# bioinfo-ut/GenomeTester4

Measured on AMD Instinct MI355X. Metric: k-mers merged/sec, 2-list k=25 intersection (glistcompare -i), lists resident in HBM, higher is better.
Workload: dtype u64 keys + u32 counts

## Files before the change

genometester4_amd/csrc/gt4hip_api.hip:

```cpp
#include "gt4hip_host.h"

#include <stdarg.h>
#include <stdio.h>
#include <stdlib.h>
#include <string.h>
#include <new>

using namespace gt4;

static thread_local char g_create_err[512] = "";

static void pool_flush (gt4hip_context *ctx);

int gt4hip_fail (gt4hip_context *ctx, int code, const char *fmt, ...)
{
  va_list ap;
  va_start (ap, fmt);
  vsnprintf (ctx ? ctx->err : g_create_err, 512, fmt, ap);
  va_end (ap);
  return code;
}

extern "C" const char *gt4hip_strerror (int code)
{
// ... 111 lines not shown
  if (!ctx) return GT4HIP_EINVAL;
  HIPCHK (ctx, hipSetDevice (ctx->device));
  HIPCHK (ctx, hipStreamSynchronize (ctx->stream));
  pool_flush (ctx);
  return GT4HIP_OK;
}

extern "C" int gt4hip_device_memory (gt4hip_context *ctx, uint64_t *free_bytes, uint64_t *total_bytes)
{
  if (!ctx) return GT4HIP_EINVAL;
  HIPCHK (ctx, hipSetDevice (ctx->device));
  size_t f = 0, t = 0;
  HIPCHK (ctx, hipMemGetInfo (&f, &t));
  if (free_bytes) *free_bytes = (uint64_t) f + ctx->pool_bytes;
  if (total_bytes) *total_bytes = (uint64_t) t;
  return GT4HIP_OK;
}

extern "C" int gt4hip_set_option (gt4hip_context *ctx, const char *name, int64_t value)
{
  if (!ctx || !name) return GT4HIP_EINVAL;
  if (!strcmp (name, "two_pass")) ctx->two_pass = value != 0;
  else if (!strcmp (name, "pool")) {
    ctx->pool_enabled = value != 0 && ctx->pool;
    if (!ctx->pool_enabled) pool_flush (ctx);
  }
  else if (!strcmp (name, "pool_cap_mb")) {
    ctx->pool_cap = value > 0 ? (size_t) value << 20 : 0;
    if (ctx->pool_bytes > ctx->pool_cap) pool_flush (ctx);
  }
  else if (!strcmp (name, "grid")) ctx->grid_override = value;
  else if (!strcmp (name, "scan_group")) ctx->scan_group = (int) value;
  else if (!strcmp (name, "dynamic")) ctx->dynamic = (int) value;
  else if (!strcmp (name, "kway")) ctx->kway_enabled = (int) value;
  else if (!strcmp (name, "kway_max")) ctx->kway_max = value == 8 ? 8 : (value == 33 ? 33 : 32);
  else if (!strcmp (name, "kway_g")) ctx->kway_g = value;
  else if (!strcmp (name, "kway_vt")) ctx->kway_vt = value;
  else if (!strcmp (name, "spin_limit")) ctx->spin_limit = value > 0 ? (uint32_t) value : 0u;
  else if (!strcmp (name, "geom1")) ctx->force_geom = value != 0 ? 1 : 0;
  else if (!strcmp (name, "geom0")) ctx->force_geom = value != 0 ? -1 : 0;
  else return gt4hip_fail (ctx, GT4HIP_EINVAL, "unknown option %s", name);
  return GT4HIP_OK;
}

extern "C" int gt4hip_get_counter (gt4hip_context *ctx, const char *name, uint64_t *value)
{
  if (!ctx || !name || !value) return GT4HIP_EINVAL;
  if (!strcmp (name, "single_pass_fallbacks")) *value = ctx->single_pass_fallbacks;
  else if (!strcmp (name, "kway_calls")) *value = ctx->kway_calls;
  else if (!strcmp (name, "kway_overflows")) *value = ctx->kway_overflows;
  else if (!strcmp (name, "kway_declined")) *value = ctx->kway_declined;
  else if (!strcmp (name, "kway_splits")) *value = ctx->kway_splits;
  else if (!strcmp (name, "kway_shared_x100")) *value = ctx->kway_shared_x100;
  else if (!strcmp (name, "kway_width")) *value = ctx->kway_width;
  else if (!strcmp (name, "nway_kernel_us")) *value = (uint64_t) (ctx->nway_kernel_ms * 1000.0);
  else if (!strcmp (name, "nway_tiles")) *value = ctx->nway_tiles;
  else if (!strcmp (name, "nway_one_pass")) *value = (uint64_t) ctx->last_multi_one_pass;
  else if (!strcmp (name, "sort_us")) *value = (uint64_t) (ctx->sort_ms * 1000.0);
  else if (!strcmp (name, "fold_us")) *value = (uint64_t) (ctx->fold_ms * 1000.0);
  else if (!strcmp (name, "extract_us")) *value = (uint64_t) (ctx->extract_ms * 1000.0);
  else if (!strcmp (name, "maker_text_tile") || !strcmp (name, "maker_code_tile")) *value = GT4HIP_MAKER_TILE;
  else if (!strcmp (name, "table_us")) *value = (uint64_t) (ctx->table_ms * 1000.0);
  else if (!strcmp (name, "query_wide")) *value = ctx->query_wide;
  else if (!strcmp (name, "mm_wide_levels")) *value = ctx->mm_wide_levels;
  else if (!strcmp (name, "mm_unskipped_levels")) *value = ctx->mm_unskipped_levels;
  else return gt4hip_fail (ctx, GT4HIP_EINVAL, "unknown counter %s", name);
// ... 310 lines not shown
```

genometester4_amd/csrc/gt4hip_device.h:

```cpp
#ifndef GT4HIP_DEVICE_H
#define GT4HIP_DEVICE_H

#include "gt4hip_internal.h"

namespace gt4 {
namespace {

constexpr int WAVE = 64;

typedef unsigned long long u64;
typedef unsigned int u32;
typedef u32 u32x4 __attribute__ ((ext_vector_type (4)));


__device__ __forceinline__ u64 load_key (const u32 *__restrict__ rec, u64 i)
{
  const u32 *p = rec + 3 * i;
  return (u64) p[0] | ((u64) p[1] << 32);
}



__device__ __forceinline__ u64 shfl_up_u64 (u64 v, int d)
{
// ... 10 lines not shown
__device__ __forceinline__ u64 wave_inclusive_scan (u64 v, int lane)
{
#pragma unroll
  for (int d = 1; d < WAVE; d <<= 1) {
    const u64 o = shfl_up_u64 (v, d);
    if (lane >= d) v += o;
  }
  return v;
}

__device__ __forceinline__ u64 wave_sum (u64 v)
{
#pragma unroll
  for (int m = WAVE / 2; m > 0; m >>= 1) v += shfl_xor_u64 (v, m);
  return v;
}

__device__ __forceinline__ u32 dpp_inclusive_scan_u32 (u32 v)
{
  v += (u32) __builtin_amdgcn_update_dpp (0, (int) v, 0x111, 0xf, 0xf, false);
  v += (u32) __builtin_amdgcn_update_dpp (0, (int) v, 0x112, 0xf, 0xf, false);
  v += (u32) __builtin_amdgcn_update_dpp (0, (int) v, 0x114, 0xf, 0xf, false);
  v += (u32) __builtin_amdgcn_update_dpp (0, (int) v, 0x118, 0xf, 0xf, false);
  v += (u32) __builtin_amdgcn_update_dpp (0, (int) v, 0x142, 0xa, 0xf, false);
  v += (u32) __builtin_amdgcn_update_dpp (0, (int) v, 0x143, 0xc, 0xf, false);
  return v;
}

__device__ __forceinline__ u32 dpp_wave_sum_u32 (u32 v)
{
  return (u32) __builtin_amdgcn_readlane ((int) dpp_inclusive_scan_u32 (v), WAVE - 1);
}

template <int NCH>
__device__ __forceinline__ u32 chunk_scan (u64 *km, u32 *cp, int lane)
{
  static_assert (NCH <= 2 * WAVE, "two chunks per lane");
  const u32 v0 = lane < NCH ? (u32) __popcll (km[lane]) : 0u;
  const u32 v1 = (NCH > WAVE && lane + WAVE < NCH) ? (u32) __popcll (km[NCH > WAVE ? lane + WAVE : 0]) : 0u;
  const u32 incl = dpp_inclusive_scan_u32 (v0 | (v1 << 16));
  const u32 last = (u32) __builtin_amdgcn_readlane ((int) incl, WAVE - 1);
  const u32 t0 = last & 0xffffu, total = t0 + (last >> 16);
  if (lane < NCH) cp[lane] = (incl & 0xffffu) - v0;
  if (NCH > WAVE && lane + WAVE < NCH) cp[lane + WAVE] = t0 + (incl >> 16) - v1;
  if (lane == 0) {
    cp[NCH] = total;
    km[NCH] = 0;
  }
  return total;
}


constexpr u32 AGG_READY = 1u << 31;
constexpr u64 CARRY_READY = 1ull << 63;

__device__ __forceinline__ void publish_u32 (u32 *p, u32 v) { __hip_atomic_store (p, v, __ATOMIC_RELAXED, __HIP_MEMORY_SCOPE_AGENT); }
__device__ __forceinline__ void publish_u64 (u64 *p, u64 v) { __hip_atomic_store (p, v, __ATOMIC_RELAXED, __HIP_MEMORY_SCOPE_AGENT); }
__device__ __forceinline__ u32 peek_u32 (u32 *p) { return __hip_atomic_load (p, __ATOMIC_RELAXED, __HIP_MEMORY_SCOPE_AGENT); }
__device__ __forceinline__ u64 peek_u64 (u64 *p) { return __hip_atomic_load (p, __ATOMIC_RELAXED, __HIP_MEMORY_SCOPE_AGENT); }

#define GT4_STAMP_TID GT4_PROFILE_PHASES
#define PHASE_STAMP(i) PROF (do { __builtin_amdgcn_sched_barrier (0); u64 t_; asm volatile ("s_memtime %0\n\ts_waitcnt lgkmcnt(0)" : "=s"(t_) :: "memory"); __builtin_amdgcn_sched_barrier (0); if (tid == GT4_STAMP_TID) { ph[i] += t_ - t_last; } t_last = t_; } while (0))

constexpr u32 SPIN_LIMIT = 1u << 22;
#define GT4_SCAN_ROWS 16
constexpr int SCAN_ROWS = GT4_SCAN_ROWS;

__device__ void scanner_wave (u32 *agg, u64 *carry_out, u64 num_tiles, PairControl *ctl, int lane, u32 spin_limit)
{
  __builtin_amdgcn_s_setprio (3);
  u64 carry = 0;
  const u64 rows = (num_tiles + WAVE - 1) / WAVE;
  if (lane == 0) publish_u64 (&carry_out[0], CARRY_READY);
  u32 v[SCAN_ROWS], w[SCAN_ROWS];
  auto load_batch = [&] (u32 (&dst)[SCAN_ROWS], u64 r0) {
#pragma unroll
    for (int j = 0; j < SCAN_ROWS; j++) {
      const u64 idx = (r0 + j) * WAVE + lane;
// ... 247 lines not shown
```

genometester4_amd/csrc/gt4hip_host.h:

```cpp
#ifndef GT4HIP_HOST_H
#define GT4HIP_HOST_H

#include "../../include/gt4hip.h"
#include "gt4hip_internal.h"

#include <stddef.h>
#include <algorithm>
#include <utility>
#include <vector>

struct gt4hip_io;

struct gt4hip_context {
  int device;
  hipStream_t stream;
  hipEvent_t ev[4];
  int n_cus;
  int two_pass;
  int64_t grid_override;
  uint32_t spin_limit;
  int dynamic;
  int scan_group;
  int force_geom;
  uint64_t single_pass_fallbacks;
  std::vector<std::pair<void *, size_t>> *pool;
  int pool_enabled;
  size_t pool_bytes;
  size_t pool_cap;
  uint64_t *part;
  size_t part_bytes;
  unsigned long long *desc;
  size_t desc_bytes;
  unsigned long long *block_sums;
  size_t block_sums_bytes;
  gt4::PairControl *ctl;
  gt4::PairControl *ctl_host;
  unsigned long long *scratch;
  unsigned long long *scratch_host;
  uint64_t *kway_part;
  size_t kway_part_bytes;
  void *kway_cnt;
  size_t kway_cnt_bytes;
  uint64_t *kway_part2;
  size_t kway_part2_bytes;
  void *kway_need;
  size_t kway_need_bytes;
  uint64_t kway_splits;
  int kway_enabled;
  int kway_max;
  uint64_t kway_width;
  uint64_t kway_shared_x100;
  int64_t kway_g;
  int64_t kway_vt;
// ... 104 lines not shown
```

genometester4_amd/csrc/gt4hip_kernels.hip:

```cpp
#define GT4_RESOLVE_LOOKBACK 3
#include "gt4hip_device.h"

#include <type_traits>

namespace gt4 {

namespace {


enum : u32 { KIND_SKIP = 0, KIND_A = 1, KIND_B = 2, KIND_BOTH = 3 };

struct StreamCoef {
  u32 m_f1, m_f2, m_min, m_max, m_sub2;
  u32 konst;
  u32 minz;
  u32 check_in;
  u32 lo;
  u32 cutoff;
  u32 subtract;
};

template <int S>
__device__ __forceinline__ StreamCoef make_coef (const PairParams &p)
{
// ... 107 lines not shown

template <int NT, int IPT, int OPS>
struct RankShared {
  static constexpr int CAP = NT * IPT;
  static constexpr int NCH = CAP / WAVE;
  static constexpr int STAGE_DW = OPS == STAGE_INTRSEC ? ((3 * (CAP / 2 + 1) + 3) & ~3)
                                  : ((OPS == STAGE_UNION || OPS == STAGE_COMPLEMENT) ? 3 * CAP
                                     : (OPS == STAGE_ANY ? 3 * (2 * CAP + 16) : (OPS == STAGE_UNION_LATE ? 3 * (CAP + 16) : 4)));
  static constexpr int STAGE_SLOTS = (OPS == STAGE_INTRSEC && IPT <= 4 && NT > 512) ? 4 : ((OPS == STAGE_ANY || OPS == STAGE_UNION_LATE) ? 1 : 2);
  alignas (16) u32 raw[3 * CAP];
  u32 stage[STAGE_SLOTS][STAGE_DW];
  u64 kmask[4][NCH + 1];
  u32 cpre[4][NCH + 1];
  u64 excl[4];
  u32 tot[4];
  u32 tick[3];
  u64 rng[3][4];
  u32 tile_id[3];
  u64 trash[WAVE];
};

__device__ __forceinline__ void store_lane0 (u64 *dst, u64 *trash, u64 v, int lane)
{
  u64 *const w = lane == 0 ? dst : trash + lane;
  *w = v;
}

__device__ __forceinline__ u32 kept_before (const u64 *km, const u32 *cp, u32 z)
{
  const u32 c = z >> 6;
  return cp[c] + (u32) __popcll (km[c] & ((1ull << (z & 63u)) - 1ull));
}

template <int S, int NT, int IPT, int OPS, int FAST, class Shared>
__device__ __forceinline__ void scatter_stream (Shared &sh, u32 *dst32, const PairParams &p, u32 nbs, int lane, int wid,
                                                const u64 (&key)[IPT], const u32 (&fa)[IPT], const u32 (&fb)[IPT], const u32 (&meta)[IPT])
{
  constexpr int NW = NT / WAVE;
  const StreamCoef c = make_coef<S> (p);
  constexpr bool A_ONLY = S == 1 || S == 2;
  const u32 pna = A_ONLY ? 0u : kept_before (sh.kmask[S], sh.cpre[S], nbs);
#pragma unroll
  for (int k = 0; k < IPT; k++) {
    const u32 chunk = (u32) k * NW + (u32) wid;
    const u64 mv = sh.kmask[S][chunk];
    const u32 m_lo = __builtin_amdgcn_readfirstlane ((u32) mv), m_hi = __builtin_amdgcn_readfirstlane ((u32) (mv >> 32));
    if (__builtin_amdgcn_inverse_ballot_w64 (((u64) m_hi << 32) | m_lo)) {
      const u32 own = sh.cpre[S][chunk] + __builtin_amdgcn_mbcnt_hi (m_hi, __builtin_amdgcn_mbcnt_lo (m_lo, 0u));
      u32 slot = own;
      if (!A_ONLY) {
        const u32 r = meta[k] & 0xffffu;
        const u32 z = ((meta[k] >> 18) & 1u) ? nbs + r : r;
        slot += kept_before (sh.kmask[S], sh.cpre[S], z) - pna;
      }
      u32 f;
      if (OPS != 0) f = fa[k];
      else if (FAST) eval_default<S> ((meta[k] >> 16) & 3u, fa[k], fb[k], p.cutoff, f);
      else eval_stream<S> ((meta[k] >> 16) & 3u, fa[k], fb[k], c, f);
      dst32[3 * slot] = (u32) key[k];
      dst32[3 * slot + 1] = (u32) (key[k] >> 32);
      dst32[3 * slot + 2] = f;
    }
  }
}

template <int CAP, int G>
__device__ __forceinline__ void rank_group (const u32 *lds32, const u32 (&sbase)[G], const u32 (&sn)[G], const u64 (&ky)[G], u32 (&lo)[G], bool narrow, u32 base_lo)
{
  auto key_at = [&] (u32 byte_off) -> u64 {
    const u32 *const q = reinterpret_cast<const u32 *> (reinterpret_cast<const char *> (lds32) + byte_off);
    return (u64) q[0] | ((u64) q[1] << 32);
  };
  constexpr u32 HTOP = (CAP & (CAP - 1)) ? (1u << (31 - __builtin_clz ((unsigned) CAP))) / 2 : CAP / 4;
  u32 at[G];
  auto step = [&] (u32 h) {
    u64 pv[G];
// ... 82 lines not shown
  for (int u = 0; u < G; u++) lo[u] = at[u] - 4u * sbase[u];
}

struct TileRange {
  u64 a0, b0;
  u32 na, nb;
};


template <int NT, int IPT, int MODE, int OPS, int FAST = 0, int OPSET = 0>
__global__ __launch_bounds__ (NT, merge_waves_per_simd (NT, MODE, OPS, FAST)) void
k_pair_merge (const u32 *__restrict__ A, u64 nA, const u32 *__restrict__ B, u64 nB, u64 *part, u64 num_tiles,
              PairParams p, PairOutputs outs, u64 *desc, PairControl *ctl)
{
  constexpr int CAP = NT * IPT;
  constexpr int NW = NT / WAVE;
  constexpr int NCH = CAP / WAVE;
  constexpr int NLOAD4 = (3 * IPT + 3) / 4;
  constexpr bool LATE1 = OPS == 1 && IPT > 4;
  constexpr bool DEFER = OPS != 0 && !LATE1 && MODE != MODE_COUNT;
  constexpr int S0 = OPS == 2 ? 1 : (OPS == 4 ? 2 : 0);
  static_assert (OPS == 0 || OPS == 1 || OPS == 2 || OPS == 4, "specialised kernels exist for one of these outputs alone");
  constexpr bool GDEFER = (OPS == 0 || LATE1) && MODE != MODE_COUNT;
  constexpr int G = IPT % 3 == 0 ? 3 : 2;
  constexpr int F_TOP = GDEFER ? NLOAD4 + 1 : (OPS == 4 ? NLOAD4 : (OPS == 2 ? 2 : 1));
  constexpr int F_MID = (GDEFER || OPS == 4 || OPS == 2) ? 0 : 1;
  constexpr bool STAGGER = NT >= 1024;
  static_assert (NW >= 4, "one wavefront per output stream in phase 2");
  static_assert (NCH <= 2 * WAVE, "chunk scan is a single wavefront pass");
  typedef RankShared<NT, IPT, (MODE == MODE_COUNT ? STAGE_NONE : (OPS == 0 ? STAGE_ANY : (OPS == 4 ? STAGE_COMPLEMENT : (OPS == 2 ? STAGE_INTRSEC : (IPT > 4 ? STAGE_UNION_LATE : STAGE_UNION)))))> Shared;
  __shared__ Shared sh;
  u32 *const lds32 = sh.raw;

  constexpr bool OPAQUE_TID = OPS == 0 && !(FAST == 1 && (OPSET == 3 || OPSET == 5) && MODE != MODE_COUNT);
  int tid = threadIdx.x, lane = tid & (WAVE - 1);
  const int wid = __builtin_amdgcn_readfirstlane (tid / WAVE);
  static_assert (pair_variant_exists ({ NT, IPT, MODE, OPS, FAST, OPSET }), "not an instantiation the selection can return (a compile-time stream set belongs to the any-combination kernel)");
  const u32 ops = OPS ? (u32) OPS : (OPSET ? (u32) OPSET : p.ops);
  const bool need_b = (ops & 9u) != 0;

  const u64 n_rows = (num_tiles + WAVE - 1) / WAVE;
  const u32 spin_limit = p.spin_limit ? p.spin_limit : SPIN_LIMIT;
  u32 *const agg = reinterpret_cast<u32 *> (desc);
  u64 *const carry = desc + 2 * n_rows * WAVE;

  u32 role = 0;
  if (MODE == MODE_LOOKBACK) {
    if (tid == 0) sh.tick[0] = atomicAdd (&ctl->role, 1u);
    __syncthreads ();
    role = sh.tick[0];
    __syncthreads ();
    if (role == 0) {
      const u32 n_str = (u32) __builtin_popcount (ops);
      const u32 k = (u32) wid % n_str, sub = (u32) wid / n_str, n_sub = ((u32) NW - k + n_str - 1) / n_str;
      u32 s = 0;
      for (u32 seen = 0, b = 0; b < 4; b++)
        if ((ops >> b) & 1u) {
          if (seen == k) s = b;
          seen++;
        }
      u64 *const rowsum = carry + 4 * (n_rows + 1);
      if (sub < 8u && (p.scan_group || sub == 0))
        scanner_part (agg + (u64) s * n_rows * WAVE, rowsum + (u64) s * n_rows, carry + (u64) s * (n_rows + 1), num_tiles, ctl, lane, spin_limit, sub,
                      p.scan_group ? (n_sub > 8u ? 8u : n_sub) : 1u);
      return;
    }
  }
// ... 148 lines not shown
    if (DEFER && w_have) {
      constexpr int WK = (Shared::STAGE_DW / 4 + NT - 1) / NT;
      write_out_fixed<NT, WK> (outs.rec[S0], uniform64 (sh.excl[S0]), w_tot, sh.stage[it % LAG], tid);
    }
    u32 xagg = 0;
    u64 xcarry = 0;
    if (GDEFER && MODE == MODE_LOOKBACK && it >= 1 && wid >= 4 && wid < 8 && ((ops >> (wid - 4)) & 1u)) {
      const int s = wid - 4;
      const u32 pt = past[LAG - 1];
      const u64 prow = pt / WAVE;
      if ((u32) lane < pt % WAVE) xagg = peek_u32 (&agg[(u64) s * n_rows * WAVE + prow * WAVE + lane]);
      xcarry = peek_u64 (&carry[(u64) s * (n_rows + 1) + prow]);
    }
    if (nxt < ntl) {
      if (STAGGER) {
#pragma unroll
        for (int j = 0; j < F_TOP; j++) fetch_part (tn, j);
      } else fetch (tn);
    }

    bool narrow = false;
    u32 base_lo = 0;
    if (OPS == 2 && MODE != MODE_COUNT && na && nb) {
      const u32 la = 3 * (na - 1), lb = OB + 3 * (nb - 1);
      const u64 a_min = (u64) lds32[0] | ((u64) lds32[1] << 32), a_max = (u64) lds32[la] | ((u64) lds32[la + 1] << 32);
      const u64 b_min = (u64) lds32[OB] | ((u64) lds32[OB + 1] << 32), b_max = (u64) lds32[lb] | ((u64) lds32[lb + 1] << 32);
      const u64 t_min = a_min < b_min ? a_min : b_min, t_max = a_max > b_max ? a_max : b_max;
      narrow = __builtin_amdgcn_ballot_w64 (((t_max - t_min) >> 32) == 0) != 0;
      base_lo = (u32) t_min;
    }
    PHASE_STAMP (2);
    u64 key[IPT];
    u32 fa[IPT], fb[IPT], meta[IPT];
    {
      const StreamCoef c0 = make_coef<0> (p), c1 = make_coef<1> (p), c2 = make_coef<2> (p), c3 = make_coef<3> (p);
      static_assert (IPT % G == 0, "chunks are searched in groups");
#pragma unroll
      for (int kk = 0; kk < IPT; kk += G) {
        if (STAGGER && kk == G && nxt < ntl) {
#pragma unroll
          for (int j = F_TOP; j < F_TOP + F_MID; j++) fetch_part (tn, j);
        }
        bool live[G], valid[G], any_live = false;
        u32 is_a[G], own[G], lim[G], lo[G];
        u32 sbase[G], sn[G];
        u32 plim[G];
        u64 ky[G];
#pragma unroll
        for (int u = 0; u < G; u++) {
          const u32 cbeg = ((u32) (kk + u) * NW + (u32) wid) * WAVE;
          is_a[u] = cbeg < nbs ? 1u : 0u;
          plim[u] = is_a[u] ? na : (need_b ? npos : 0u);
          live[u] = cbeg < plim[u];
          any_live |= live[u];
        }
        if (!any_live) {
#pragma unroll
          for (int u = 0; u < G; u++) {
            const int k = kk + u;
            key[k] = 0;
            fa[k] = fb[k] = 0;
            meta[k] = KIND_SKIP << 16;
            {
              const u32 chunk = (u32) k * NW + (u32) wid;
#pragma unroll
              for (int s = 0; s < 4; s++)
                if ((ops >> s) & 1u) store_lane0 (&sh.kmask[s][chunk], sh.trash, 0ull, lane);
            }
          }
          continue;
        }
#pragma unroll
        for (int u = 0; u < G; u++) {
          const u32 e = (u32) (kk + u) * NT + (u32) tid;
          u32 at;
          if (OPS == 2) {
            valid[u] = live[u] && (is_a[u] ? e < na : e < npos);
            at = valid[u] ? (is_a[u] ? 3 * e : OB + 3 * (e - nbs)) : 0u;
          } else {
            valid[u] = e < plim[u];
            const u32 off = is_a[u] ? 0u : OB - 3 * nbs;
            at = valid[u] ? 3 * e + off : 0u;
          }
          ky[u] = (u64) lds32[at] | ((u64) lds32[at + 1] << 32);
          own[u] = lds32[at + 2];
          sbase[u] = is_a[u] ? OB : 0u;
          sn[u] = is_a[u] ? nb : na;
          lim[u] = valid[u] ? 12 * sn[u] : 0u;
          lo[u] = 0;
        }
        rank_group<CAP, G> (lds32, sbase, sn, ky, lo, narrow, base_lo);
#pragma unroll
        for (int u = 0; u < G; u++) {
          const int k = kk + u;
          const u32 chunk = (u32) k * NW + (u32) wid;
          const u32 r = (lo[u] * 43691u) >> 19;
          const bool in = lo[u] < lim[u];
          const u32 oat = sbase[u] + (in ? lo[u] >> 2 : 0u);
          const u64 okey = (u64) lds32[oat] | ((u64) lds32[oat + 1] << 32);
          const u32 ocnt = lds32[oat + 2];
          const bool matched = in & (okey == ky[u]);
          if (FAST && (OPS == 2 || OPS == 4)) {
            u32 f;
            bool keep;
            if (OPS == 2 && FAST == 1) {
              f = own[u] < ocnt ? own[u] : ocnt;
              keep = matched && f >= (p.cutoff ? p.cutoff : 1u);
            } else if (OPS == 2) {
              const u32 mn = own[u] < ocnt ? own[u] : ocnt;
              f = own[u] == 0u ? ocnt : mn;
              keep = matched && (FAST == 2 || f >= p.cutoff);
            } else {
              const u32 xb = matched ? ocnt : 0u;
              f = own[u] - xb;
              keep = valid[u] && own[u] >= p.cutoff && xb < p.cutoff && f != 0u;
            }
            key[k] = ky[u];
            fa[k] = f;
            fb[k] = 0;
            meta[k] = 0;
            const u64 m = __builtin_amdgcn_ballot_w64 (keep);
            store_lane0 (&sh.kmask[OPS == 2 ? 1 : 2][chunk], sh.trash, m, lane);
            if (OPS == 2) acc_sum1 += keep ? f : 0u;
            else acc_sum2 += keep ? f : 0u;
            continue;
          }
          if (FAST && OPS == 1) {
            const u32 xo = (is_a[u] && matched) ? ocnt : 0u;
            const u32 f = own[u] + xo;
            const bool keep = valid[u] && (is_a[u] || !matched) &&
                              (FAST == 2 || (FAST == 3 ? f >= p.cutoff : ((own[u] >= p.cutoff || xo >= p.cutoff) && f != 0u)));
            key[k] = ky[u];
            fa[k] = f;
            fb[k] = 0;
            meta[k] = r | (is_a[u] << 18);
            const u64 m = __builtin_amdgcn_ballot_w64 (keep);
            sh.kmask[0][chunk] = m;
            acc_sum0 += keep ? f : 0u;
            continue;
          }
          u32 kind, xa, xb;
          if (is_a[u]) {
            kind = matched ? KIND_BOTH : KIND_A;
            xa = own[u];
            xb = matched ? ocnt : 0u;
          } else {
            kind = matched ? KIND_SKIP : KIND_B;
            xa = 0;
            xb = own[u];
          }
          if (!valid[u]) kind = KIND_SKIP;
          key[k] = ky[u];
          fa[k] = xa;
          fb[k] = xb;
          meta[k] = (OPS == 2 || OPS == 4) ? 0u : (r | (kind << 16) | (is_a[u] << 18));
          u32 f;
          if (ops & 1u) {
            const bool keep = (FAST && OPS == 0) ? eval_default<0> (kind, xa, xb, p.cutoff, f) : eval_stream<0> (kind, xa, xb, c0, f);
            const u64 m = __builtin_amdgcn_ballot_w64 (keep);
            sh.kmask[0][chunk] = m;
            acc_sum0 += keep ? f : 0u;
          }
          if ((!FAST || OPS == 0) && (ops & 2u)) {
            const bool keep = (FAST && OPS == 0) ? eval_default<1> (kind, xa, xb, p.cutoff, f) : eval_stream<1> (kind, xa, xb, c1, f);
            const u64 m = __builtin_amdgcn_ballot_w64 (keep);
            sh.kmask[1][chunk] = m;
            acc_sum1 += keep ? f : 0u;
          }
          if ((!FAST || OPS == 0) && (ops & 4u)) {
            const bool keep = (FAST && OPS == 0) ? eval_default<2> (kind, xa, xb, p.cutoff, f) : eval_stream<2> (kind, xa, xb, c2, f);
            const u64 m = __builtin_amdgcn_ballot_w64 (keep);
            sh.kmask[2][chunk] = m;
            acc_sum2 += keep ? f : 0u;
          }
          if ((!FAST || OPS == 0) && (ops & 8u)) {
            const bool keep = (FAST && OPS == 0) ? eval_default<3> (kind, xa, xb, p.cutoff, f) : eval_stream<3> (kind, xa, xb, c3, f);
            const u64 m = __builtin_amdgcn_ballot_w64 (keep);
            sh.kmask[3][chunk] = m;
            acc_sum3 += keep ? f : 0u;
          }
          if (OPS != 0) fa[k] = f;
        }
      }
    }
#pragma unroll
    for (int k = 0; k < IPT; k++) {
      if (OPS == 0) asm volatile ("" : "+v"(fa[k]), "+v"(fb[k]), "+v"(meta[k]));
      else if (OPS == 1) asm volatile ("" : "+v"(fa[k]), "+v"(meta[k]));
      else asm volatile ("" : "+v"(fa[k]));
    }
    if (GDEFER && it >= 1 && wid >= 4 && wid < 8 && ((ops >> (wid - 4)) & 1u)) {
      const int s = wid - 4;
      const u32 pt = past[LAG - 1];
      u64 x;
      if (MODE == MODE_LOOKBACK) x = resolve_offset (agg + (u64) s * n_rows * WAVE, carry + (u64) s * (n_rows + 1), pt, lane, xagg, xcarry, ctl, spin_limit);
      else x = desc[4 * (u64) pt + s];
      if (lane == 0) sh.excl[s] = 12 * x;
    }
    if (STAGGER && nxt < ntl) {
#pragma unroll
      for (int j = (G == IPT ? F_TOP : F_TOP + F_MID); j <= NLOAD4; j++) fetch_part (tn, j);
    }
    if (DEFER && n_have && wid == 4) {
      if (MODE == MODE_LOOKBACK) {
        const u64 prow = n_tile / WAVE;
        dagg = 0;
        if ((u32) lane < n_tile % WAVE) dagg = peek_u32 (&agg[(u64) S0 * n_rows * WAVE + prow * WAVE + lane]);
        dcarry = peek_u64 (&carry[(u64) S0 * (n_rows + 1) + prow]);
      } else {
        dcarry = __hip_atomic_load (&desc[4 * (u64) n_tile + S0], __ATOMIC_RELAXED, __HIP_MEMORY_SCOPE_AGENT);
      }
    }
    PHASE_STAMP (3);
    __syncthreads ();
    PHASE_STAMP (4);

    u32 my_total = 0;
    if (DEFER) {
      my_total = chunk_scan<NCH> (sh.kmask[S0], sh.cpre[S0], lane);
      blk_cnt += my_total;
      if (wid == 0 && MODE == MODE_LOOKBACK) {
        if (lane == 0) publish_u32 (&agg[(u64) S0 * n_rows * WAVE + cur], AGG_READY | my_total);
      }
    }
    if (!DEFER && wid < 4 && ((ops >> wid) & 1u)) {
      const int s = wid;
      const u32 total = chunk_scan<NCH> (sh.kmask[s], sh.cpre[s], lane);
      if (lane == 0) {
        sh.tot[s] = total;
        blk_cnt += total;
        if (MODE == MODE_COUNT) {
          if (desc) desc[4 * (u64) cur + s] = total;
        } else if (MODE == MODE_LOOKBACK) {
          publish_u32 (&agg[(u64) s * n_rows * WAVE + cur], AGG_READY | total);
        }
      }
    }

    PHASE_STAMP (5);
    if (GDEFER) {
      if (it >= 1) {
#pragma unroll
        for (int s = 0; s < 4; s++)
          if ((ops >> s) & 1u) write_out_fixed<NT, (3 * CAP / 4 + NT - 1) / NT> (outs.rec[s], uniform64 (sh.excl[s]), g_tot[s], sh.stage[0] + 3 * g_off[s], tid);
      }
      __syncthreads ();
      u32 run = 0;
#pragma unroll
      for (int s = 0; s < 4; s++) {
        g_off[s] = run;
        g_tot[s] = ((ops >> s) & 1u) ? uniform32 (sh.tot[s]) : 0u;
        run += (g_tot[s] + 3u) & ~3u;
      }
#pragma unroll
      for (int s = 0; s < 4; s++) {
        if (!((ops >> s) & 1u)) continue;
        u32 *const dst = sh.stage[0] + 3 * g_off[s];
        switch (s) {
          case 0: scatter_stream<0, NT, IPT, OPS, FAST> (sh, dst, p, nbs, lane, wid, key, fa, fb, meta); break;
          case 1: scatter_stream<1, NT, IPT, OPS, FAST> (sh, dst, p, nbs, lane, wid, key, fa, fb, meta); break;
          case 2: scatter_stream<2, NT, IPT, OPS, FAST> (sh, dst, p, nbs, lane, wid, key, fa, fb, meta); break;
          default: scatter_stream<3, NT, IPT, OPS, FAST> (sh, dst, p, nbs, lane, wid, key, fa, fb, meta); break;
        }
      }
    } else if (DEFER) {
      u32 *const slot = sh.stage[it % LAG];
      const u32 my_tot = my_total;
      scatter_stream<S0, NT, IPT, OPS, FAST> (sh, slot, p, nbs, lane, wid, key, fa, fb, meta);
#pragma unroll
      for (int q = 0; q + 1 < LAG; q++) pend_tot[q] = pend_tot[q + 1];
      pend_tot[LAG - 1] = my_tot;
    }
    PHASE_STAMP (6);
    if (tid == 0) {
      sh.tile_id[s_nn] = hk_tile;
      if (hk_have_rng) {
        {
          sh.rng[s_nn][0] = 12 * hk_rng[0];
          sh.rng[s_nn][1] = 12 * hk_rng[1];
          sh.rng[s_nn][2] = hk_rng[2] - hk_rng[0];
          sh.rng[s_nn][3] = hk_rng[3] - hk_rng[1];
        }
      }
    }
#pragma unroll
    for (int q = 0; q + 1 < LAG; q++) past[q] = past[q + 1];
    past[LAG - 1] = cur;
    PHASE_STAMP (7);
    cur = nxt;
    tr = tn;
    it++;
    {
      const int r_cur = r_nxt;
      r_nxt = r_nn;
      r_nn = r_cur == 0 ? 2 : r_cur - 1;
    }
  }
PROF (
  if (tid == GT4_STAMP_TID)
    for (int i = 0; i < 8; i++) atomicAdd (&ctl->phase_cycles[i], ph[i]);
)

  if (GDEFER && it >= 1) {
    const u32 pt = past[LAG - 1];
    __syncthreads ();
// ... 301 lines not shown
```

genometester4_amd/csrc/gt4hip_pair.hip:

```cpp
#include "gt4hip_host.h"

#include <stdio.h>
#include <string.h>

using namespace gt4;

size_t gt4hip_lookback_desc_bytes (uint64_t tiles)
{
  const uint64_t rows = (tiles + 63) / 64;
  return (((size_t) rows * 64 * 16 + (size_t) (rows + 1) * 32 + (size_t) rows * 32) + 255) & ~(size_t) 255;
}

static size_t desc_bytes_for (uint64_t tiles)
{
  const size_t two = ((size_t) tiles * 32 + 255) & ~(size_t) 255;
  return std::max (gt4hip_lookback_desc_bytes (tiles), two);
}

int gt4hip_run_pair (gt4hip_context *ctx, const uint32_t *A, uint64_t nA, const uint32_t *B, uint64_t nB, const PairParams &p_in,
                     bool count_only, uint32_t *const dst[4], PairRun *run, bool force_two_pass)
{
  if (p_in.ops == 8u) {
    PairParams q = p_in;
    q.ops = 4u;
    q.rule[2] = p_in.rule[3];
    q.subtract = 0;
    uint32_t *const d2[4] = { NULL, NULL, dst ? dst[3] : NULL, NULL };
    const int rc = gt4hip_run_pair (ctx, B, nB, A, nA, q, count_only, d2, run, force_two_pass);
    run->n_words[3] = run->n_words[2];
    run->total_count[3] = run->total_count[2];
    run->n_words[2] = run->total_count[2] = 0;
    return rc;
  }
  if (p_in.ops == 2u && nA > nB && p_in.rule[1] != 2u && p_in.rule[1] != RULE_MINZ) {
    PairParams q = p_in;
    if (q.rule[1] == 5u) q.rule[1] = 6u;
    else if (q.rule[1] == 6u) q.rule[1] = 5u;
    return gt4hip_run_pair (ctx, B, nB, A, nA, q, count_only, dst, run, force_two_pass);
  }
  PairParams p = p_in;
  p.spin_limit = ctx->spin_limit;
  memset (run, 0, sizeof *run);
  const uint64_t total = nA + nB;
  if (!total || !p.ops) return GT4HIP_OK;
  const bool two_pass = (ctx->two_pass || force_two_pass) && !count_only;
  const int geom = ctx->force_geom ? (ctx->force_geom > 0 ? 1 : 0) : (count_only ? 0 : 1);
  const PairVariant v1 = pair_variant (geom, (count_only || two_pass) ? MODE_COUNT : MODE_LOOKBACK, p);
  const PairVariant v2 = pair_variant (geom, MODE_OFFSETS, p);
  const uint64_t tile_records = merge_tile_records (v1);
  const uint64_t tiles = (total + tile_records - 1) / tile_records;
  if (tiles >= 0xffffffffull) return gt4hip_fail (ctx, GT4HIP_EINVAL, "lists too long: %llu merge tiles", (unsigned long long) tiles);
  run->tiles = tiles;
  p.dynamic = ctx->dynamic > 0 ? 1u : (ctx->dynamic < 0 ? 0u : ((geom == 1 && !count_only && p.ops != 4u && p.ops != 8u) ? 1u : 0u));
  p.scan_group = ctx->scan_group > 0 ? 1u : (ctx->scan_group < 0 ? 0u : (tiles > (20000ull << 6) ? 1u : 0u));
  int rc;
  if ((rc = gt4hip_grow (ctx, (void **) &ctx->part, &ctx->part_bytes, (size_t) (tiles + 1) * 16 + (size_t) (tiles / 64 + 3) * 8))) return rc;
  const bool need_desc = !count_only;
  if (need_desc && (rc = gt4hip_grow (ctx, (void **) &ctx->desc, &ctx->desc_bytes, desc_bytes_for (tiles)))) return rc;
  if (two_pass) {
    const size_t nb = (size_t) ((tiles + 2047) / 2048) * 32;
    if ((rc = gt4hip_grow (ctx, (void **) &ctx->block_sums, &ctx->block_sums_bytes, nb))) return rc;
  }
  int grid = ctx->n_cus * merge_blocks_per_cu (v1);
  if (ctx->grid_override > 0) grid = (int) ctx->grid_override;
  if ((uint64_t) grid > tiles + 1) grid = (int) tiles + 1;
  int grid2 = ctx->n_cus * merge_blocks_per_cu (v2);
  if ((uint64_t) grid2 > tiles) grid2 = (int) tiles;

  PairOutputs outs;
  for (int s = 0; s < 4; s++) outs.rec[s] = (count_only || !dst) ? NULL : dst[s];

  hipStream_t st = ctx->stream;
  HIPCHK (ctx, hipEventRecord (ctx->ev[0], st));
  HIPCHK (ctx, hipMemsetAsync (ctx->ctl, 0, sizeof (PairControl), st));
// ... 116 lines not shown
```

genometester4_amd/csrc/gt4hip_pair_variant.h:

```cpp
#ifndef GT4HIP_PAIR_VARIANT_H
#define GT4HIP_PAIR_VARIANT_H

#include <stdint.h>

namespace gt4 {

constexpr uint32_t RULE_MINZ = 8;

enum Filter : uint32_t {
  FILTER_REFERENCE = 0,
  FILTER_RAW = 1,
  FILTER_RESULT = 2
};

struct PairParams {
  uint32_t ops;
  uint32_t rule[4];
  uint32_t cutoff;
  uint32_t subtract;
  uint32_t count_override;
  uint32_t filter;
  uint32_t spin_limit;
  uint32_t scan_group;
  uint32_t dynamic;
};

enum MergeMode : int {
  MODE_COUNT = 0,
  MODE_LOOKBACK = 1,
  MODE_OFFSETS = 2
};

constexpr int MERGE_VT = 4;
constexpr int MERGE_TILE_SLACK = 64;

constexpr int GT4_IPT_UNION = 4;
constexpr int GT4_IPT_INTERSECT = 6;
constexpr int GT4_IPT_INTERSECT_SMALL = 4;

constexpr int merge_waves_per_simd (int nt, int mode, int ops = 0, int fast = 0)
{
  return (nt == 512 && (mode == MODE_COUNT || (ops == 2 && fast == 1 && GT4_IPT_INTERSECT_SMALL <= 4))) ? 6 : 4;
}

constexpr int merge_ipt (int nt, int ops_class)
{
  return (nt == 1024 && ops_class == 2) ? GT4_IPT_INTERSECT
         : ((nt == 1024 && ops_class == 1) ? GT4_IPT_UNION : ((nt == 512 && ops_class == 2) ? GT4_IPT_INTERSECT_SMALL : MERGE_VT));
}

struct PairVariant {
  int nt, ipt, mode, cls, fast, opset;
};

constexpr bool opset_geometry (int nt, int mode) { return mode == MODE_COUNT ? nt == 512 : nt == 1024; }

constexpr bool pair_variant_exists (const PairVariant &v)
// ... 34 lines not shown
```

Baseline: 355.9 billion.

## Rank and scatter only A-side rows in single-pass intersection/subtract kernels

For A-only operations (intersection, subtract) in lookback mode, when the tile's A part fits in half the per-thread items, the rank, mask-scan and scatter loops cover only the first IPT/2 rows instead of all IPT. B-side rows contribute nothing to these outputs, so the change is meant to cut the binary-search and ballot work on them. The chunk scan skips writing its sentinel on this path. This adds a runtime branch that instantiates two versions of the body, which raises code size and may raise register pressure. An option can turn the path off.

```diff
diff --git a/genometester4_amd/csrc/gt4hip_api.hip b/genometester4_amd/csrc/gt4hip_api.hip
--- a/genometester4_amd/csrc/gt4hip_api.hip
+++ b/genometester4_amd/csrc/gt4hip_api.hip
@@ -167,6 +167,7 @@
   else if (!strcmp (name, "grid")) ctx->grid_override = value;
   else if (!strcmp (name, "scan_group")) ctx->scan_group = (int) value;
   else if (!strcmp (name, "dynamic")) ctx->dynamic = (int) value;
+  else if (!strcmp (name, "a_rows")) ctx->a_rows = (int) value;
   else if (!strcmp (name, "kway")) ctx->kway_enabled = (int) value;
   else if (!strcmp (name, "kway_max")) ctx->kway_max = value == 8 ? 8 : (value == 33 ? 33 : 32);
   else if (!strcmp (name, "kway_g")) ctx->kway_g = value;
diff --git a/genometester4_amd/csrc/gt4hip_device.h b/genometester4_amd/csrc/gt4hip_device.h
--- a/genometester4_amd/csrc/gt4hip_device.h
+++ b/genometester4_amd/csrc/gt4hip_device.h
@@ -66,7 +66,7 @@
   return (u32) __builtin_amdgcn_readlane ((int) dpp_inclusive_scan_u32 (v), WAVE - 1);
 }
 
-template <int NCH>
+template <int NCH, bool SENTINEL = true>
 __device__ __forceinline__ u32 chunk_scan (u64 *km, u32 *cp, int lane)
 {
   static_assert (NCH <= 2 * WAVE, "two chunks per lane");
@@ -77,7 +77,7 @@
   const u32 t0 = last & 0xffffu, total = t0 + (last >> 16);
   if (lane < NCH) cp[lane] = (incl & 0xffffu) - v0;
   if (NCH > WAVE && lane + WAVE < NCH) cp[lane + WAVE] = t0 + (incl >> 16) - v1;
-  if (lane == 0) {
+  if (SENTINEL && lane == 0) {
     cp[NCH] = total;
     km[NCH] = 0;
   }
diff --git a/genometester4_amd/csrc/gt4hip_host.h b/genometester4_amd/csrc/gt4hip_host.h
--- a/genometester4_amd/csrc/gt4hip_host.h
+++ b/genometester4_amd/csrc/gt4hip_host.h
@@ -19,6 +19,7 @@
   int two_pass;
   int64_t grid_override;
   uint32_t spin_limit;
+  int a_rows;
   int dynamic;
   int scan_group;
   int force_geom;
diff --git a/genometester4_amd/csrc/gt4hip_kernels.hip b/genometester4_amd/csrc/gt4hip_kernels.hip
--- a/genometester4_amd/csrc/gt4hip_kernels.hip
+++ b/genometester4_amd/csrc/gt4hip_kernels.hip
@@ -163,7 +163,7 @@
   return cp[c] + (u32) __popcll (km[c] & ((1ull << (z & 63u)) - 1ull));
 }
 
-template <int S, int NT, int IPT, int OPS, int FAST, class Shared>
+template <int S, int NT, int IPT, int KR, int OPS, int FAST, class Shared>
 __device__ __forceinline__ void scatter_stream (Shared &sh, u32 *dst32, const PairParams &p, u32 nbs, int lane, int wid,
                                                 const u64 (&key)[IPT], const u32 (&fa)[IPT], const u32 (&fb)[IPT], const u32 (&meta)[IPT])
 {
@@ -172,7 +172,7 @@
   constexpr bool A_ONLY = S == 1 || S == 2;
   const u32 pna = A_ONLY ? 0u : kept_before (sh.kmask[S], sh.cpre[S], nbs);
 #pragma unroll
-  for (int k = 0; k < IPT; k++) {
+  for (int k = 0; k < KR; k++) {
     const u32 chunk = (u32) k * NW + (u32) wid;
     const u64 mv = sh.kmask[S][chunk];
     const u32 m_lo = __builtin_amdgcn_readfirstlane ((u32) mv), m_hi = __builtin_amdgcn_readfirstlane ((u32) (mv >> 32));
@@ -321,7 +321,9 @@
   __shared__ Shared sh;
   u32 *const lds32 = sh.raw;
 
-  constexpr bool OPAQUE_TID = OPS == 0 && !(FAST == 1 && (OPSET == 3 || OPSET == 5) && MODE != MODE_COUNT);
+  constexpr bool A_ROWS = (OPS == 2 || OPS == 4) && MODE == MODE_LOOKBACK;
+  constexpr int KA = IPT / 2;
+  constexpr bool OPAQUE_TID = A_ROWS || (OPS == 0 && !(FAST == 1 && (OPSET == 3 || OPSET == 5) && MODE != MODE_COUNT));
   int tid = threadIdx.x, lane = tid & (WAVE - 1);
   const int wid = __builtin_amdgcn_readfirstlane (tid / WAVE);
   static_assert (pair_variant_exists ({ NT, IPT, MODE, OPS, FAST, OPSET }), "not an instantiation the selection can return (a compile-time stream set belongs to the any-combination kernel)");
@@ -536,163 +538,173 @@
     PHASE_STAMP (2);
     u64 key[IPT];
     u32 fa[IPT], fb[IPT], meta[IPT];
-    {
-      const StreamCoef c0 = make_coef<0> (p), c1 = make_coef<1> (p), c2 = make_coef<2> (p), c3 = make_coef<3> (p);
-      static_assert (IPT % G == 0, "chunks are searched in groups");
-#pragma unroll
-      for (int kk = 0; kk < IPT; kk += G) {
-        if (STAGGER && kk == G && nxt < ntl) {
-#pragma unroll
-          for (int j = F_TOP; j < F_TOP + F_MID; j++) fetch_part (tn, j);
-        }
-        bool live[G], valid[G], any_live = false;
-        u32 is_a[G], own[G], lim[G], lo[G];
-        u32 sbase[G], sn[G];
-        u32 plim[G];
-        u64 ky[G];
-#pragma unroll
-        for (int u = 0; u < G; u++) {
-          const u32 cbeg = ((u32) (kk + u) * NW + (u32) wid) * WAVE;
-          is_a[u] = cbeg < nbs ? 1u : 0u;
-          plim[u] = is_a[u] ? na : (need_b ? npos : 0u);
-          live[u] = cbeg < plim[u];
-          any_live |= live[u];
-        }
-        if (!any_live) {
+    auto rank_rows = [&] (auto rows) __attribute__ ((always_inline)) {
+      constexpr int KR = decltype (rows)::value;
+      constexpr bool AROWS = KR < IPT;
+      static_assert (!AROWS || (A_ROWS && DEFER), "the A-rows body belongs to the single-pass A-only kernels");
+      {
+        const StreamCoef c0 = make_coef<0> (p), c1 = make_coef<1> (p), c2 = make_coef<2> (p), c3 = make_coef<3> (p);
+        static_assert (KR % G == 0, "chunks are searched in groups");
+#pragma unroll
+        for (int kk = 0; kk < KR; kk += G) {
+          if (STAGGER && kk == G && nxt < ntl) {
+#pragma unroll
+            for (int j = F_TOP; j < F_TOP + F_MID; j++) fetch_part (tn, j);
+          }
+          bool live[G], valid[G], any_live = false;
+          u32 is_a[G], own[G], lim[G], lo[G];
+          u32 sbase[G], sn[G];
+          u32 plim[G];
+          u64 ky[G];
+#pragma unroll
+          for (int u = 0; u < G; u++) {
+            const u32 cbeg = ((u32) (kk + u) * NW + (u32) wid) * WAVE;
+            is_a[u] = AROWS ? 1u : (cbeg < nbs ? 1u : 0u);
+            plim[u] = is_a[u] ? na : (need_b ? npos : 0u);
+            live[u] = AROWS ? true : cbeg < plim[u];
+            any_live |= live[u];
+          }
+          if (!AROWS && !any_live) {
+#pragma unroll
+            for (int u = 0; u < G; u++) {
+              const int k = kk + u;
+              key[k] = 0;
+              fa[k] = fb[k] = 0;
+              meta[k] = KIND_SKIP << 16;
+              {
+                const u32 chunk = (u32) k * NW + (u32) wid;
+#pragma unroll
+                for (int s = 0; s < 4; s++)
+                  if ((ops >> s) & 1u) store_lane0 (&sh.kmask[s][chunk], sh.trash, 0ull, lane);
+              }
+            }
+            continue;
+          }
+#pragma unroll
+          for (int u = 0; u < G; u++) {
+            const u32 e = (u32) (kk + u) * NT + (u32) tid;
+            u32 at;
+            if (OPS == 2) {
+              valid[u] = live[u] && (is_a[u] ? e < na : e < npos);
+              at = valid[u] ? (is_a[u] ? 3 * e : OB + 3 * (e - nbs)) : 0u;
+            } else {
+              valid[u] = e < plim[u];
+              const u32 off = is_a[u] ? 0u : OB - 3 * nbs;
+              at = valid[u] ? 3 * e + off : 0u;
+            }
+            ky[u] = (u64) lds32[at] | ((u64) lds32[at + 1] << 32);
+            own[u] = lds32[at + 2];
+            sbase[u] = is_a[u] ? OB : 0u;
+            sn[u] = is_a[u] ? nb : na;
+            lim[u] = valid[u] ? 12 * sn[u] : 0u;
+            lo[u] = 0;
+          }
+          rank_group<CAP, G> (lds32, sbase, sn, ky, lo, narrow, base_lo);
 #pragma unroll
           for (int u = 0; u < G; u++) {
             const int k = kk + u;
-            key[k] = 0;
-            fa[k] = fb[k] = 0;
-            meta[k] = KIND_SKIP << 16;
-            {
-              const u32 chunk = (u32) k * NW + (u32) wid;
-#pragma unroll
-              for (int s = 0; s < 4; s++)
-                if ((ops >> s) & 1u) store_lane0 (&sh.kmask[s][chunk], sh.trash, 0ull, lane);
+            const u32 chunk = (u32) k * NW + (u32) wid;
+            const u32 r = (lo[u] * 43691u) >> 19;
+            const bool in = lo[u] < lim[u];
+            const u32 oat = sbase[u] + (in ? lo[u] >> 2 : 0u);
+            const u64 okey = (u64) lds32[oat] | ((u64) lds32[oat + 1] << 32);
+            const u32 ocnt = lds32[oat + 2];
+            const bool matched = in & (okey == ky[u]);
+            if (FAST && (OPS == 2 || OPS == 4)) {
+              u32 f;
+              bool keep;
+              if (OPS == 2 && FAST == 1) {
+                f = own[u] < ocnt ? own[u] : ocnt;
+                keep = matched && f >= (p.cutoff ? p.cutoff : 1u);
+              } else if (OPS == 2) {
+                const u32 mn = own[u] < ocnt ? own[u] : ocnt;
+                f = own[u] == 0u ? ocnt : mn;
+                keep = matched && (FAST == 2 || f >= p.cutoff);
+              } else {
+                const u32 xb = matched ? ocnt : 0u;
+                f = own[u] - xb;
+                keep = valid[u] && own[u] >= p.cutoff && xb < p.cutoff && f != 0u;
+              }
+              key[k] = ky[u];
+              fa[k] = f;
+              fb[k] = 0;
+              meta[k] = 0;
+              const u64 m = __builtin_amdgcn_ballot_w64 (keep);
+              store_lane0 (&sh.kmask[OPS == 2 ? 1 : 2][chunk], sh.trash, m, lane);
+              if (OPS == 2) acc_sum1 += keep ? f : 0u;
+              else acc_sum2 += keep ? f : 0u;
+              continue;
             }
+            if (FAST && OPS == 1) {
+              const u32 xo = (is_a[u] && matched) ? ocnt : 0u;
+              const u32 f = own[u] + xo;
+              const bool keep = valid[u] && (is_a[u] || !matched) &&
+                                (FAST == 2 || (FAST == 3 ? f >= p.cutoff : ((own[u] >= p.cutoff || xo >= p.cutoff) && f != 0u)));
+              key[k] = ky[u];
+              fa[k] = f;
+              fb[k] = 0;
+              meta[k] = r | (is_a[u] << 18);
+              const u64 m = __builtin_amdgcn_ballot_w64 (keep);
+              sh.kmask[0][chunk] = m;
+              acc_sum0 += keep ? f : 0u;
+              continue;
+            }
+            u32 kind, xa, xb;
+            if (is_a[u]) {
+              kind = matched ? KIND_BOTH : KIND_A;
+              xa = own[u];
+              xb = matched ? ocnt : 0u;
+            } else {
+              kind = matched ? KIND_SKIP : KIND_B;
+              xa = 0;
+              xb = own[u];
+            }
+            if (!valid[u]) kind = KIND_SKIP;
+            key[k] = ky[u];
+            fa[k] = xa;
+            fb[k] = xb;
+            meta[k] = (OPS == 2 || OPS == 4) ? 0u : (r | (kind << 16) | (is_a[u] << 18));
+            u32 f;
+            if (ops & 1u) {
+              const bool keep = (FAST && OPS == 0) ? eval_default<0> (kind, xa, xb, p.cutoff, f) : eval_stream<0> (kind, xa, xb, c0, f);
+              const u64 m = __builtin_amdgcn_ballot_w64 (keep);
+              sh.kmask[0][chunk] = m;
+              acc_sum0 += keep ? f : 0u;
+            }
+            if ((!FAST || OPS == 0) && (ops & 2u)) {
+              const bool keep = (FAST && OPS == 0) ? eval_default<1> (kind, xa, xb, p.cutoff, f) : eval_stream<1> (kind, xa, xb, c1, f);
+              const u64 m = __builtin_amdgcn_ballot_w64 (keep);
+              sh.kmask[1][chunk] = m;
+              acc_sum1 += keep ? f : 0u;
+            }
+            if ((!FAST || OPS == 0) && (ops & 4u)) {
+              const bool keep = (FAST && OPS == 0) ? eval_default<2> (kind, xa, xb, p.cutoff, f) : eval_stream<2> (kind, xa, xb, c2, f);
+              const u64 m = __builtin_amdgcn_ballot_w64 (keep);
+              sh.kmask[2][chunk] = m;
+              acc_sum2 += keep ? f : 0u;
+            }
+            if ((!FAST || OPS == 0) && (ops & 8u)) {
+              const bool keep = (FAST && OPS == 0) ? eval_default<3> (kind, xa, xb, p.cutoff, f) : eval_stream<3> (kind, xa, xb, c3, f);
+              const u64 m = __builtin_amdgcn_ballot_w64 (keep);
+              sh.kmask[3][chunk] = m;
+              acc_sum3 += keep ? f : 0u;
+            }
+            if (OPS != 0) fa[k] = f;
           }
-          continue;
         }
-#pragma unroll
-        for (int u = 0; u < G; u++) {
-          const u32 e = (u32) (kk + u) * NT + (u32) tid;
-          u32 at;
-          if (OPS == 2) {
-            valid[u] = live[u] && (is_a[u] ? e < na : e < npos);
-            at = valid[u] ? (is_a[u] ? 3 * e : OB + 3 * (e - nbs)) : 0u;
-          } else {
-            valid[u] = e < plim[u];
-            const u32 off = is_a[u] ? 0u : OB - 3 * nbs;
-            at = valid[u] ? 3 * e + off : 0u;
-          }
-          ky[u] = (u64) lds32[at] | ((u64) lds32[at + 1] << 32);
-          own[u] = lds32[at + 2];
-          sbase[u] = is_a[u] ? OB : 0u;
-          sn[u] = is_a[u] ? nb : na;
-          lim[u] = valid[u] ? 12 * sn[u] : 0u;
-          lo[u] = 0;
-        }
-        rank_group<CAP, G> (lds32, sbase, sn, ky, lo, narrow, base_lo);
-#pragma unroll
-        for (int u = 0; u < G; u++) {
-          const int k = kk + u;
-          const u32 chunk = (u32) k * NW + (u32) wid;
-          const u32 r = (lo[u] * 43691u) >> 19;
-          const bool in = lo[u] < lim[u];
-          const u32 oat = sbase[u] + (in ? lo[u] >> 2 : 0u);
-          const u64 okey = (u64) lds32[oat] | ((u64) lds32[oat + 1] << 32);
-          const u32 ocnt = lds32[oat + 2];
-          const bool matched = in & (okey == ky[u]);
-          if (FAST && (OPS == 2 || OPS == 4)) {
-            u32 f;
-            bool keep;
-            if (OPS == 2 && FAST == 1) {
-              f = own[u] < ocnt ? own[u] : ocnt;
-              keep = matched && f >= (p.cutoff ? p.cutoff : 1u);
-            } else if (OPS == 2) {
-              const u32 mn = own[u] < ocnt ? own[u] : ocnt;
-              f = own[u] == 0u ? ocnt : mn;
-              keep = matched && (FAST == 2 || f >= p.cutoff);
-            } else {
-              const u32 xb = matched ? ocnt : 0u;
-              f = own[u] - xb;
-              keep = valid[u] && own[u] >= p.cutoff && xb < p.cutoff && f != 0u;
-            }
-            key[k] = ky[u];
-            fa[k] = f;
-            fb[k] = 0;
-            meta[k] = 0;
-            const u64 m = __builtin_amdgcn_ballot_w64 (keep);
-            store_lane0 (&sh.kmask[OPS == 2 ? 1 : 2][chunk], sh.trash, m, lane);
-            if (OPS == 2) acc_sum1 += keep ? f : 0u;
-            else acc_sum2 += keep ? f : 0u;
-            continue;
-          }
-          if (FAST && OPS == 1) {
-            const u32 xo = (is_a[u] && matched) ? ocnt : 0u;
-            const u32 f = own[u] + xo;
-            const bool keep = valid[u] && (is_a[u] || !matched) &&
-                              (FAST == 2 || (FAST == 3 ? f >= p.cutoff : ((own[u] >= p.cutoff || xo >= p.cutoff) && f != 0u)));
-            key[k] = ky[u];
-            fa[k] = f;
-            fb[k] = 0;
-            meta[k] = r | (is_a[u] << 18);
-            const u64 m = __builtin_amdgcn_ballot_w64 (keep);
-            sh.kmask[0][chunk] = m;
-            acc_sum0 += keep ? f : 0u;
-            continue;
-          }
-          u32 kind, xa, xb;
-          if (is_a[u]) {
-            kind = matched ? KIND_BOTH : KIND_A;
-            xa = own[u];
-            xb = matched ? ocnt : 0u;
-          } else {
-            kind = matched ? KIND_SKIP : KIND_B;
-            xa = 0;
-            xb = own[u];
-          }
-          if (!valid[u]) kind = KIND_SKIP;
-          key[k] = ky[u];
-          fa[k] = xa;
-          fb[k] = xb;
-          meta[k] = (OPS == 2 || OPS == 4) ? 0u : (r | (kind << 16) | (is_a[u] << 18));
-          u32 f;
-          if (ops & 1u) {
-            const bool keep = (FAST && OPS == 0) ? eval_default<0> (kind, xa, xb, p.cutoff, f) : eval_stream<0> (kind, xa, xb, c0, f);
-            const u64 m = __builtin_amdgcn_ballot_w64 (keep);
-            sh.kmask[0][chunk] = m;
-            acc_sum0 += keep ? f : 0u;
-          }
-          if ((!FAST || OPS == 0) && (ops & 2u)) {
-            const bool keep = (FAST && OPS == 0) ? eval_default<1> (kind, xa, xb, p.cutoff, f) : eval_stream<1> (kind, xa, xb, c1, f);
-            const u64 m = __builtin_amdgcn_ballot_w64 (keep);
-            sh.kmask[1][chunk] = m;
-            acc_sum1 += keep ? f : 0u;
-          }
-          if ((!FAST || OPS == 0) && (ops & 4u)) {
-            const bool keep = (FAST && OPS == 0) ? eval_default<2> (kind, xa, xb, p.cutoff, f) : eval_stream<2> (kind, xa, xb, c2, f);
-            const u64 m = __builtin_amdgcn_ballot_w64 (keep);
-            sh.kmask[2][chunk] = m;
-            acc_sum2 += keep ? f : 0u;
-          }
-          if ((!FAST || OPS == 0) && (ops & 8u)) {
-            const bool keep = (FAST && OPS == 0) ? eval_default<3> (kind, xa, xb, p.cutoff, f) : eval_stream<3> (kind, xa, xb, c3, f);
-            const u64 m = __builtin_amdgcn_ballot_w64 (keep);
-            sh.kmask[3][chunk] = m;
-            acc_sum3 += keep ? f : 0u;
-          }
-          if (OPS != 0) fa[k] = f;
-        }
-      }
-    }
-#pragma unroll
-    for (int k = 0; k < IPT; k++) {
-      if (OPS == 0) asm volatile ("" : "+v"(fa[k]), "+v"(fb[k]), "+v"(meta[k]));
-      else if (OPS == 1) asm volatile ("" : "+v"(fa[k]), "+v"(meta[k]));
-      else asm volatile ("" : "+v"(fa[k]));
-    }
+      }
+#pragma unroll
+      for (int k = 0; k < KR; k++) {
+        if (OPS == 0) asm volatile ("" : "+v"(fa[k]), "+v"(fb[k]), "+v"(meta[k]));
+        else if (OPS == 1) asm volatile ("" : "+v"(fa[k]), "+v"(meta[k]));
+        else asm volatile ("" : "+v"(fa[k]));
+      }
+    };
+    const bool a_body = A_ROWS && !p.a_rows_off && na <= (u32) (NT * KA);
+    if constexpr (A_ROWS) {
+      if (a_body) rank_rows (std::integral_constant<int, KA>{});
+      else rank_rows (std::integral_constant<int, IPT>{});
+    } else rank_rows (std::integral_constant<int, IPT>{});
     if (GDEFER && it >= 1 && wid >= 4 && wid < 8 && ((ops >> (wid - 4)) & 1u)) {
       const int s = wid - 4;
       const u32 pt = past[LAG - 1];
@@ -718,63 +730,70 @@
     PHASE_STAMP (3);
     __syncthreads ();
     PHASE_STAMP (4);
-
-    u32 my_total = 0;
-    if (DEFER) {
-      my_total = chunk_scan<NCH> (sh.kmask[S0], sh.cpre[S0], lane);
-      blk_cnt += my_total;
-      if (wid == 0 && MODE == MODE_LOOKBACK) {
-        if (lane == 0) publish_u32 (&agg[(u64) S0 * n_rows * WAVE + cur], AGG_READY | my_total);
-      }
-    }
-    if (!DEFER && wid < 4 && ((ops >> wid) & 1u)) {
-      const int s = wid;
-      const u32 total = chunk_scan<NCH> (sh.kmask[s], sh.cpre[s], lane);
-      if (lane == 0) {
-        sh.tot[s] = total;
-        blk_cnt += total;
-        if (MODE == MODE_COUNT) {
-          if (desc) desc[4 * (u64) cur + s] = total;
-        } else if (MODE == MODE_LOOKBACK) {
-          publish_u32 (&agg[(u64) s * n_rows * WAVE + cur], AGG_READY | total);
+    auto stage_rows = [&] (auto rows) __attribute__ ((always_inline)) {
+      constexpr int KR = decltype (rows)::value;
+      constexpr bool AROWS = KR < IPT;
+      u32 my_total = 0;
+      if (DEFER) {
+        my_total = chunk_scan<KR * NW, !AROWS> (sh.kmask[S0], sh.cpre[S0], lane);
+        blk_cnt += my_total;
+        if (wid == 0 && MODE == MODE_LOOKBACK) {
+          if (lane == 0) publish_u32 (&agg[(u64) S0 * n_rows * WAVE + cur], AGG_READY | my_total);
         }
       }
-    }
-
-    PHASE_STAMP (5);
-    if (GDEFER) {
-      if (it >= 1) {
-#pragma unroll
-        for (int s = 0; s < 4; s++)
-          if ((ops >> s) & 1u) write_out_fixed<NT, (3 * CAP / 4 + NT - 1) / NT> (outs.rec[s], uniform64 (sh.excl[s]), g_tot[s], sh.stage[0] + 3 * g_off[s], tid);
-      }
-      __syncthreads ();
-      u32 run = 0;
-#pragma unroll
-      for (int s = 0; s < 4; s++) {
-        g_off[s] = run;
-        g_tot[s] = ((ops >> s) & 1u) ? uniform32 (sh.tot[s]) : 0u;
-        run += (g_tot[s] + 3u) & ~3u;
-      }
-#pragma unroll
-      for (int s = 0; s < 4; s++) {
-        if (!((ops >> s) & 1u)) continue;
-        u32 *const dst = sh.stage[0] + 3 * g_off[s];
-        switch (s) {
-          case 0: scatter_stream<0, NT, IPT, OPS, FAST> (sh, dst, p, nbs, lane, wid, key, fa, fb, meta); break;
-          case 1: scatter_stream<1, NT, IPT, OPS, FAST> (sh, dst, p, nbs, lane, wid, key, fa, fb, meta); break;
-          case 2: scatter_stream<2, NT, IPT, OPS, FAST> (sh, dst, p, nbs, lane, wid, key, fa, fb, meta); break;
-          default: scatter_stream<3, NT, IPT, OPS, FAST> (sh, dst, p, nbs, lane, wid, key, fa, fb, meta); break;
+      if (!DEFER && wid < 4 && ((ops >> wid) & 1u)) {
+        const int s = wid;
+        const u32 total = chunk_scan<NCH> (sh.kmask[s], sh.cpre[s], lane);
+        if (lane == 0) {
+          sh.tot[s] = total;
+          blk_cnt += total;
+          if (MODE == MODE_COUNT) {
+            if (desc) desc[4 * (u64) cur + s] = total;
+          } else if (MODE == MODE_LOOKBACK) {
+            publish_u32 (&agg[(u64) s * n_rows * WAVE + cur], AGG_READY | total);
+          }
         }
       }
-    } else if (DEFER) {
-      u32 *const slot = sh.stage[it % LAG];
-      const u32 my_tot = my_total;
-      scatter_stream<S0, NT, IPT, OPS, FAST> (sh, slot, p, nbs, lane, wid, key, fa, fb, meta);
-#pragma unroll
-      for (int q = 0; q + 1 < LAG; q++) pend_tot[q] = pend_tot[q + 1];
-      pend_tot[LAG - 1] = my_tot;
-    }
+
+      PHASE_STAMP (5);
+      if (GDEFER) {
+        if (it >= 1) {
+#pragma unroll
+          for (int s = 0; s < 4; s++)
+            if ((ops >> s) & 1u) write_out_fixed<NT, (3 * CAP / 4 + NT - 1) / NT> (outs.rec[s], uniform64 (sh.excl[s]), g_tot[s], sh.stage[0] + 3 * g_off[s], tid);
+        }
+        __syncthreads ();
+        u32 run = 0;
+#pragma unroll
+        for (int s = 0; s < 4; s++) {
+          g_off[s] = run;
+          g_tot[s] = ((ops >> s) & 1u) ? uniform32 (sh.tot[s]) : 0u;
+          run += (g_tot[s] + 3u) & ~3u;
+        }
+#pragma unroll
+        for (int s = 0; s < 4; s++) {
+          if (!((ops >> s) & 1u)) continue;
+          u32 *const dst = sh.stage[0] + 3 * g_off[s];
+          switch (s) {
+            case 0: scatter_stream<0, NT, IPT, KR, OPS, FAST> (sh, dst, p, nbs, lane, wid, key, fa, fb, meta); break;
+            case 1: scatter_stream<1, NT, IPT, KR, OPS, FAST> (sh, dst, p, nbs, lane, wid, key, fa, fb, meta); break;
+            case 2: scatter_stream<2, NT, IPT, KR, OPS, FAST> (sh, dst, p, nbs, lane, wid, key, fa, fb, meta); break;
+            default: scatter_stream<3, NT, IPT, KR, OPS, FAST> (sh, dst, p, nbs, lane, wid, key, fa, fb, meta); break;
+          }
+        }
+      } else if (DEFER) {
+        u32 *const slot = sh.stage[it % LAG];
+        const u32 my_tot = my_total;
+        scatter_stream<S0, NT, IPT, KR, OPS, FAST> (sh, slot, p, nbs, lane, wid, key, fa, fb, meta);
+#pragma unroll
+        for (int q = 0; q + 1 < LAG; q++) pend_tot[q] = pend_tot[q + 1];
+        pend_tot[LAG - 1] = my_tot;
+      }
+    };
+    if constexpr (A_ROWS) {
+      if (a_body) stage_rows (std::integral_constant<int, KA>{});
+      else stage_rows (std::integral_constant<int, IPT>{});
+    } else stage_rows (std::integral_constant<int, IPT>{});
     PHASE_STAMP (6);
     if (tid == 0) {
       sh.tile_id[s_nn] = hk_tile;
diff --git a/genometester4_amd/csrc/gt4hip_pair.hip b/genometester4_amd/csrc/gt4hip_pair.hip
--- a/genometester4_amd/csrc/gt4hip_pair.hip
+++ b/genometester4_amd/csrc/gt4hip_pair.hip
@@ -40,6 +40,7 @@
   }
   PairParams p = p_in;
   p.spin_limit = ctx->spin_limit;
+  p.a_rows_off = ctx->a_rows < 0 ? 1u : 0u;
   memset (run, 0, sizeof *run);
   const uint64_t total = nA + nB;
   if (!total || !p.ops) return GT4HIP_OK;
diff --git a/genometester4_amd/csrc/gt4hip_pair_variant.h b/genometester4_amd/csrc/gt4hip_pair_variant.h
--- a/genometester4_amd/csrc/gt4hip_pair_variant.h
+++ b/genometester4_amd/csrc/gt4hip_pair_variant.h
@@ -23,6 +23,7 @@
   uint32_t spin_limit;
   uint32_t scan_group;
   uint32_t dynamic;
+  uint32_t a_rows_off;
 };
 
 enum MergeMode : int {
```

Measured after the change: 366.7 billion, median of 6. 3.0% higher.
